# Zoz4/Pooraytracer

Hardware: AMD Instinct MI355X
Metric: Mrays/s (primary+secondary) at fixed spp; s/frame in ms_per_step (higher is better)
Workload: dtype f64; 1 GPU; cornell-box (synthetic stand-in, 20492 tris, 4-wide BVH 6148 nodes) 1024x1024 spp=500 depth=20 rr=0.8 bSampleLights seed=1; parallelism=32x32 tiles dealt diagonally over 1 GPU(s), rays_per_frame=2362685805

## Files before the change

pooraytracer_amd/csrc/prt_device.h:

```cpp
#pragma once
#include <hip/hip_runtime.h>
#include <stdint.h>

#include "prt_types.h"
#include "prt_light_pick.h"

#define PRT_DEV __device__ __forceinline__
typedef prt_real real;
#define PRT_F32 (sizeof(prt_real) == 4)
#define RL(x) ((real)(x))
template <typename R> struct real4_of;
template <> struct real4_of<double> { typedef double4 type; };
template <> struct real4_of<float> { typedef float4 type; };
typedef real4_of<real>::type real4;
#define PRT_NOCUR ((int32_t)0x80000000)
#ifndef PRT_BOX_PK
#define PRT_BOX_PK 1
#endif
#ifndef PRT_LEAF_BATCH
#define PRT_LEAF_BATCH 32
#endif
#ifndef PRT_INNER_MIN
#define PRT_INNER_MIN 12
#endif

struct d3 {
    real x, y, z;
};
struct d2 {
    real x, y;
};
PRT_DEV d3 mk3(real x, real y, real z) { return d3{x, y, z}; }
PRT_DEV d3 ld3(const real* p) { return d3{p[0], p[1], p[2]}; }
PRT_DEV d3 operator+(d3 a, d3 b) { return {a.x + b.x, a.y + b.y, a.z + b.z}; }
PRT_DEV d3 operator-(d3 a, d3 b) { return {a.x - b.x, a.y - b.y, a.z - b.z}; }
PRT_DEV d3 operator-(d3 a) { return {-a.x, -a.y, -a.z}; }
PRT_DEV d3 operator*(d3 a, d3 b) { return {a.x * b.x, a.y * b.y, a.z * b.z}; }
PRT_DEV d3 operator*(d3 a, real s) { return {a.x * s, a.y * s, a.z * s}; }
PRT_DEV d3 operator*(real s, d3 a) { return {s * a.x, s * a.y, s * a.z}; }
PRT_DEV d3 operator/(d3 a, real s);
PRT_DEV real dot(d3 a, d3 b) { return a.x * b.x + a.y * b.y + a.z * b.z; }
PRT_DEV d3 cross(d3 x, d3 y) { return {x.y * y.z - y.y * x.z, x.z * y.x - y.z * x.x, x.x * y.y - y.x * x.y}; }
PRT_DEV double fast_rsqrt(double x) {
    const double y = __builtin_amdgcn_rsq(x);
    const double g = x * y, h = 0.5 * y;
    const double r = fma(-h, g, 0.5);
    const double h1 = fma(h, r, h), g1 = fma(g, r, g);
    const double e = fma(-h1, g1, 0.5);
    return 2.0 * fma(h1, e, h1);
}
PRT_DEV double fast_sqrt(double x) {
    const double y = __builtin_amdgcn_rsq(x);
    const double g = x * y, h = 0.5 * y;
    const double r = fma(-h, g, 0.5);
    const double g1 = fma(g, r, g), h1 = fma(h, r, h);
    const double d = fma(-g1, g1, x);
    const double s = fma(d, h1, g1);
    return x == 0.0 ? 0.0 : s;
}
PRT_DEV double fast_rcp(double b) {
    double r = __builtin_amdgcn_rcp(b);
    r = fma(fma(-b, r, 1.0), r, r);
    r = fma(fma(-b, r, 1.0), r, r);
    return r;
}
PRT_DEV double fast_div(double a, double b) {
    const double r = fast_rcp(b);
    const double q = a * r;
    return fma(fma(-b, q, a), r, q);
}
PRT_DEV float fast_rsqrt(float x) { return __builtin_amdgcn_rsqf(x); }
PRT_DEV float fast_sqrt(float x) { return __builtin_amdgcn_sqrtf(x); }
PRT_DEV float fast_rcp(float b) { return __builtin_amdgcn_rcpf(b); }
PRT_DEV float fast_div(float a, float b) { return a * __builtin_amdgcn_rcpf(b); }
PRT_DEV double ieee_sqrt(double x) { return sqrt(x); }
PRT_DEV float ieee_sqrt(float x) { return __builtin_amdgcn_sqrtf(x); }
PRT_DEV double ieee_div(double a, double b) { return a / b; }
PRT_DEV float ieee_div(float a, float b) { return a * __builtin_amdgcn_rcpf(b); }
PRT_DEV d3 operator/(d3 a, real s) {
    const real r = fast_rcp(s);
    return {a.x * r, a.y * r, a.z * r};
}
PRT_DEV real length(d3 v) { return fast_sqrt(dot(v, v)); }
PRT_DEV d3 normalize(d3 v) { return v * fast_rsqrt(dot(v, v)); }
PRT_DEV d3 normalize_len(d3 v, real& len) {
    const real q = dot(v, v);
    const real inv = fast_rsqrt(q);
    len = q * inv;
    return v * inv;
}

#define PRT_PI RL(3.14159265358979323846)
#define PRT_INV_PI RL(0.31830988618379067154)
#define PRT_INV_2PI RL(0.15915494309189533577)
#define PRT_PI_OVER_2 RL(1.57079632679489661923)
#define PRT_PI_OVER_4 RL(0.78539816339744830961)
#define PRT_INF RL(__builtin_huge_val())

PRT_DEV uint64_t mix64(uint64_t z) {
    z ^= z >> 30;
    z *= 0xBF58476D1CE4E5B9ULL;
    z ^= z >> 27;
    z *= 0x94D049BB133111EBULL;
    z ^= z >> 31;
    return z;
}
PRT_DEV uint64_t seed_key(uint64_t seed) { return mix64(seed + 0x9E3779B97F4A7C15ULL); }
struct Rng {
    uint64_t s;
    PRT_DEV void seed_keyed(uint64_t key, uint64_t pixel, uint64_t sample) {
        s = mix64(((uint64_t)((uint32_t)(key >> 32) ^ (uint32_t)(pixel + 1)) << 32) | ((uint32_t)key ^ (uint32_t)(sample + 1)));
        if (s == 0) s = 0x9E3779B97F4A7C15ULL;
    }
    PRT_DEV void seed(uint64_t seed, uint64_t pixel, uint64_t sample) { seed_keyed(seed_key(seed), pixel, sample); }
    PRT_DEV real next() {
        uint32_t s0 = (uint32_t)s, s1 = (uint32_t)(s >> 32);
        const uint32_t r = s0 * 0x9E3779BBu;
        s1 ^= s0;
        s0 = __builtin_amdgcn_alignbit(s0, s0, 6) ^ s1 ^ (s1 << 9);
        s1 = __builtin_amdgcn_alignbit(s1, s1, 19);
        s = ((uint64_t)s1 << 32) | s0;
        if (PRT_F32) return (real)(r >> 8) * RL(5.9604644775390625e-8);
        return (real)(r >> 1) * (RL(1.0) / RL(2147483648.0));
    }
};

struct HitInfo {
    real t;
    real alpha, beta;
    int32_t tri;
};

struct WorkCount {
    uint32_t nodes, tris;
    uint32_t tris_full;
    uint32_t inner_rounds, leaf_rounds;
};

template <bool PAD>
PRT_DEV const DTri* tri_at(const DScene& S, uint32_t i) {
    return reinterpret_cast<const DTri*>(reinterpret_cast<const char*>(S.tris) + (size_t)i * (PAD ? PRT_TRI_PAD_STRIDE(real) : (uint32_t)sizeof(DTri)));
}

PRT_DEV bool tri_test(const DTri* __restrict__ T, d3 o, d3 d, real tmin, real tmax, real& t_out, real& a_out,
                      real& b_out, const real4* pre = nullptr, uint32_t* n_full = nullptr) {
    const real4* q = reinterpret_cast<const real4*>(T);
    real4 q0 = pre ? *pre : q[0], q1 = q[1];
    d3 n = mk3(q0.x, q0.y, q0.z);
    real denom = dot(n, d);
    if (fabs(denom) < RL(1e-8)) return false;
    real t = ieee_div(q0.w - dot(n, o), denom);
    if (!(tmin <= t && t <= tmax)) return false;
    if (n_full) ++*n_full;
    const real4 q2 = q[2];
    const d3 p = o + d * t;
    const real alpha = (p.x * q1.x + p.y * q1.y + p.z * q1.z) - q1.w;
    const real beta = (p.x * q2.x + p.y * q2.y + p.z * q2.z) - q2.w;
    if (alpha != alpha || beta != beta) return false;
    if ((alpha < 0) || (beta < 0) || (alpha + beta > 1)) return false;
    t_out = t;
    a_out = alpha;
    b_out = beta;
    return true;
}

PRT_DEV float f32_up(real x) {
    const float f = (float)x;
    return f + fabsf(f) * 2.4e-7f;
}
PRT_DEV float f32_down(real x) {
    const float f = (float)x;
    return f - fabsf(f) * 2.4e-7f;
}

struct SlabAxis {
    float idq, c_lo, c_hi;
    uint32_t rot;
};
PRT_DEV SlabAxis slab_axis(real o, real d, float E, float g0, float gs) {
    SlabAxis a;
    const float df = (float)d;
    float id = __builtin_amdgcn_rcpf(df);
    if (!(fabsf(id) <= 1e28f)) id = copysignf(1e28f, df);
    const float r = (float)((real)g0 - o);
    const float c = r * id;
    const float pad = fmaf(E, fabsf(id), fabsf(c)) * 9.5367432e-7f;
    a.idq = gs * id;
    a.c_lo = c - pad;
    a.c_hi = c + pad;
    a.rot = id >= 0.f ? 0u : 16u;
    return a;
}

template <bool PAD, bool PK = false>
struct Trav {
    d3 o, d;
    real tmin;
    HitInfo hit;
    SlabAxis ax, ay, az;
    float tminf, tbestf;
    int32_t cur;
    int32_t sp;
    bool active;

    PRT_DEV void init(const DScene& S, d3 o_, d3 d_, real tmin_, real tmax_) {
        o = o_;
        d = d_;
        start(S, tmin_, tmax_);
    }
    PRT_DEV void start(const DScene& S, real tmin_, real tmax_) {
        tmin = tmin_;
        ax = slab_axis(o.x, d.x, S.slab_scale, S.grid_origin[0], S.grid_step[0]);
        ay = slab_axis(o.y, d.y, S.slab_scale, S.grid_origin[1], S.grid_step[1]);
        az = slab_axis(o.z, d.z, S.slab_scale, S.grid_origin[2], S.grid_step[2]);
        tminf = f32_down(tmin_);
        tbestf = f32_up(tmax_);
        hit.t = tmax_;
        hit.tri = -1;
        sp = 0;
        cur = 0;
        active = S.n_tris != 0;
    }

    PRT_DEV void box4(uint32_t x, uint32_t y, uint32_t z, float& n, float& f) const {
        x = __builtin_amdgcn_alignbit(x, x, ax.rot);
        y = __builtin_amdgcn_alignbit(y, y, ay.rot);
        z = __builtin_amdgcn_alignbit(z, z, az.rot);
        float nx, fx, ny, fy, nz, fz;
        if (PK) {
        typedef float f2_ __attribute__((ext_vector_type(2)));
        const f2_ tx = __builtin_elementwise_fma(f2_{(float)(x & 0xffffu), (float)(x >> 16)}, f2_{ax.idq, ax.idq}, f2_{ax.c_lo, ax.c_hi});
        const f2_ ty = __builtin_elementwise_fma(f2_{(float)(y & 0xffffu), (float)(y >> 16)}, f2_{ay.idq, ay.idq}, f2_{ay.c_lo, ay.c_hi});
        const f2_ tz = __builtin_elementwise_fma(f2_{(float)(z & 0xffffu), (float)(z >> 16)}, f2_{az.idq, az.idq}, f2_{az.c_lo, az.c_hi});
        nx = tx.x, fx = tx.y, ny = ty.x, fy = ty.y, nz = tz.x, fz = tz.y;
        } else {
        nx = fmaf((float)(x & 0xffffu), ax.idq, ax.c_lo), fx = fmaf((float)(x >> 16), ax.idq, ax.c_hi);
        ny = fmaf((float)(y & 0xffffu), ay.idq, ay.c_lo), fy = fmaf((float)(y >> 16), ay.idq, ay.c_hi);
        nz = fmaf((float)(z & 0xffffu), az.idq, az.c_lo), fz = fmaf((float)(z >> 16), az.idq, az.c_hi);
        }
        n = fmaxf(fmaxf(fmaxf(nx, ny), nz), tminf);
        f = fminf(fminf(fminf(fx, fy), fz), tbestf);
    }
    template <bool COUNT>
    PRT_DEV void inner_step(const DScene& S, uint32_t* stk, WorkCount& wc) {
        const uint4* np = reinterpret_cast<const uint4*>(S.nodes + cur);
        const uint4 bx = np[0], by = np[1], bz = np[2], rf = np[3];
        if (COUNT) wc.nodes++;
        float n0, f0, n1, f1, n2, f2, n3, f3;
        box4(bx.x, by.x, bz.x, n0, f0);
        box4(bx.y, by.y, bz.y, n1, f1);
        box4(bx.z, by.z, bz.z, n2, f2);
        box4(bx.w, by.w, bz.w, n3, f3);
        uint32_t k0 = n0 <= f0 ? __float_as_uint(n0) : 0xffffffffu;
        uint32_t k1 = n1 <= f1 ? __float_as_uint(n1) : 0xffffffffu;
        uint32_t k2 = (n2 <= f2 && rf.z != 0x80000000u) ? __float_as_uint(n2) : 0xffffffffu;
        uint32_t k3 = (n3 <= f3 && rf.w != 0x80000000u) ? __float_as_uint(n3) : 0xffffffffu;
        uint32_t r0 = rf.x, r1 = rf.y, r2 = rf.z, r3 = rf.w;
#define PRT_CE(ka, ra, kb, rb)                  \
    {                                           \
        const bool sw_ = kb < ka;               \
        const uint32_t tk_ = sw_ ? kb : ka;     \
        kb = sw_ ? ka : kb;                     \
        ka = tk_;                               \
        const uint32_t tr_ = sw_ ? rb : ra;     \
        rb = sw_ ? ra : rb;                     \
        ra = tr_;                               \
    }
        PRT_CE(k0, r0, k1, r1)
        PRT_CE(k2, r2, k3, r3)
        PRT_CE(k0, r0, k2, r2)
        PRT_CE(k1, r1, k3, r3)
        PRT_CE(k1, r1, k2, r2)
#undef PRT_CE
        if (k3 != 0xffffffffu) {
            stk[sp * 64] = r3;
            sp++;
        }
        if (k2 != 0xffffffffu) {
            stk[sp * 64] = r2;
            sp++;
        }
        if (k1 != 0xffffffffu) {
            stk[sp * 64] = r1;
            sp++;
        }
        if (k0 != 0xffffffffu) {
            cur = (int32_t)r0;
        } else if (sp == 0) {
            cur = PRT_NOCUR;
        } else {
            sp--;
            cur = (int32_t)stk[sp * 64];
        }
        if (cur == PRT_NOCUR) active = false;
    }

    template <bool COUNT>
    PRT_DEV bool test_leaf(const DScene& S, int32_t ref, WorkCount& wc, real tmin_use, bool any_hit) {
        const uint32_t enc = ~(uint32_t)ref;
        const uint32_t first = enc >> 3, cnt = (enc & 7u) + 1u;
        bool stop = false;
        real4 q0n = *reinterpret_cast<const real4*>(tri_at<PAD>(S, first));
        for (uint32_t i = 0; i < cnt; ++i) {
            real t, al, be;
            if (COUNT) wc.tris++;
            const real4 q0c = q0n;
            if (i + 1 < cnt) q0n = *reinterpret_cast<const real4*>(tri_at<PAD>(S, first + i + 1));
            if (tri_test(tri_at<PAD>(S, first + i), o, d, tmin_use, hit.t, t, al, be, &q0c, COUNT ? &wc.tris_full : nullptr)) {
                hit.t = t;
                if (!any_hit) {
                    hit.alpha = al;
                    hit.beta = be;
                }
                hit.tri = (int32_t)(first + i);
                tbestf = f32_up(t);
                if (any_hit) stop = true;
            }
        }
        return stop;
    }

    template <bool COUNT>
    PRT_DEV void leaf_step(const DScene& S, uint32_t* stk, WorkCount& wc, real tmin_use, bool any_hit) {
        bool stop = false;
        if (cur < 0 && cur != PRT_NOCUR) {
            stop = test_leaf<COUNT>(S, cur, wc, tmin_use, any_hit);
            cur = PRT_NOCUR;
        }
        if (stop) {
            active = false;
        } else if (cur == PRT_NOCUR) {
            if (sp == 0) active = false;
            else {
                sp--;
                cur = (int32_t)stk[sp * 64];
            }
        }
    }

    template <bool COUNT>
    PRT_DEV void round(const DScene& S, uint32_t* stk, WorkCount& wc, int leaf_batch, int inner_min, real tmin_use,
                       bool any_hit) {
        if (COUNT && __ballot(active && cur >= 0) != 0ULL) wc.inner_rounds++;
        if (active && cur >= 0) inner_step<COUNT>(S, stk, wc);
        const bool parked = active && cur < 0;
        const bool has_leaf = active && cur < 0 && cur != PRT_NOCUR;
        const int n_parked = __popcll(__ballot(parked));
        const int n_inner = __popcll(__ballot(active && cur >= 0));
        if (n_parked >= leaf_batch || n_inner <= inner_min) {
            if (COUNT && __ballot(has_leaf) != 0ULL) wc.leaf_rounds++;
            if (has_leaf) leaf_step<COUNT>(S, stk, wc, tmin_use, any_hit);
        }
    }
};

PRT_DEV int wave_count(bool p) { return __popcll(__ballot(p)); }

#define PRT_TEX_QUAD_REALS 16
template <bool EXTRA, bool NARROW = false>
PRT_DEV d3 tex_value(const DScene& S, int ti, real u, real v) {
    const DTexture tx = S.textures[ti];
    if (!tx.has_data) return mk3(RL(0.), RL(1.), RL(1.));
    u = fmin(fmax(u, RL(0.0)), RL(1.0));
    v = fmin(fmax(v, RL(0.0)), RL(1.0));
    real x = u * (tx.width - RL(1.));
    real y = (RL(1.) - v) * (tx.height - RL(1.));
    int x0 = (int)x, y0 = (int)y;
    real fx = x - x0, fy = y - y0;
    d3 c00, c10, c01, c11;
    if (!EXTRA || !S.tex_compact) {
        const real4* q = reinterpret_cast<const real4*>(S.texels_lin + tx.offset + (size_t)(y0 * tx.width + x0) * PRT_TEX_QUAD_REALS);
        if (NARROW) {
            const real4 r0 = q[0], r1 = q[1];
            const d3 top = mk3(r0.x, r0.y, r0.z) * (1 - fx) + mk3(r0.w, r1.x, r1.y) * fx;
            __builtin_amdgcn_sched_barrier(0);
            const real4 r2 = q[2];
            const d3 bot = mk3(r1.z, r1.w, r2.x) * (1 - fx) + mk3(r2.y, r2.z, r2.w) * fx;
            return top * (1 - fy) + bot * fy;
        }
        const real4 q0 = q[0], q1 = q[1], q2 = q[2];
        c00 = mk3(q0.x, q0.y, q0.z), c10 = mk3(q0.w, q1.x, q1.y);
        c01 = mk3(q1.z, q1.w, q2.x), c11 = mk3(q2.y, q2.z, q2.w);
    } else {
        const int x1 = min(x0 + 1, tx.width - 1), y1 = min(y0 + 1, tx.height - 1);
        const real* base = S.texels_lin + tx.offset;
        if (NARROW) {
            const d3 top = ld3(base + ((size_t)y0 * tx.width + x0) * 3) * (1 - fx) + ld3(base + ((size_t)y0 * tx.width + x1) * 3) * fx;
            __builtin_amdgcn_sched_barrier(0);
            const d3 bot = ld3(base + ((size_t)y1 * tx.width + x0) * 3) * (1 - fx) + ld3(base + ((size_t)y1 * tx.width + x1) * 3) * fx;
            return top * (1 - fy) + bot * fy;
        }
        c00 = ld3(base + ((size_t)y0 * tx.width + x0) * 3), c10 = ld3(base + ((size_t)y0 * tx.width + x1) * 3);
        c01 = ld3(base + ((size_t)y1 * tx.width + x0) * 3), c11 = ld3(base + ((size_t)y1 * tx.width + x1) * 3);
    }
    d3 c0 = c00 * (1 - fx) + c10 * fx;
    d3 c1 = c01 * (1 - fx) + c11 * fx;
    return c0 * (1 - fy) + c1 * fy;
}

PRT_DEV double fma_ks(double a, double b, double k) {
#if defined(__HIP_DEVICE_COMPILE__)
    double r;
    asm("v_fma_f64 %0, %1, %2, %3" : "=v"(r) : "v"(a), "v"(b), "s"(k));
    return r;
#else
    return __builtin_fma(a, b, k);
#endif
}
PRT_DEV float fma_ks(float a, float b, float k) { return __builtin_fmaf(a, b, k); }
PRT_DEV double fma_sk(double a, double k, double c) {
#if defined(__HIP_DEVICE_COMPILE__)
    double r;
    asm("v_fma_f64 %0, %1, %2, %3" : "=v"(r) : "v"(a), "s"(k), "v"(c));
    return r;
#else
    return __builtin_fma(a, k, c);
#endif
}
PRT_DEV double mul_ks(double a, double k) {
#if defined(__HIP_DEVICE_COMPILE__)
    double r;
    asm("v_mul_f64 %0, %1, %2" : "=v"(r) : "v"(a), "s"(k));
    return r;
#else
    return a * k;
#endif
}

PRT_DEV void sincos_quarter(real x, real& sn, real& cs) {
    const real z = x * x;
    if (PRT_F32) {
        sn = x + (x * z) * (RL(-1.6666667e-01) + z * (RL(8.3333333e-03) + z * (RL(-1.9841270e-04) + z * RL(2.7557319e-06))));
        cs = RL(1.0) + z * (RL(-0.5) + z * (RL(4.1666667e-02) + z * (RL(-1.3888889e-03) + z * RL(2.4801587e-05))));
        return;
    }
    real ps = fma_ks(z, RL(1.58969099521155010221e-10), -RL(2.50507602534068634195e-08));
    ps = fma_ks(z, ps, RL(2.75573137070700676789e-06));
    ps = fma_ks(z, ps, -RL(1.98412698298579493134e-04));
    ps = fma_ks(z, ps, RL(8.33333333332248946124e-03));
    sn = x + (x * z) * fma_ks(z, ps, -RL(1.66666666666666324348e-01));
    real pc = fma_ks(z, -RL(1.13596475577881948265e-11), RL(2.08757232129817482790e-09));
    pc = fma_ks(z, pc, -RL(2.75573143513906633035e-07));
    pc = fma_ks(z, pc, RL(2.48015872894767294178e-05));
    pc = fma_ks(z, pc, -RL(1.38888888888741095749e-03));
    pc = z * fma_ks(z, pc, RL(4.16666666666666019037e-02));
    cs = RL(1.0) - (RL(0.5) * z - z * pc);
}
PRT_DEV void sincos_turns(real u, real& sn, real& cs) {
    const real k = floor(RL(4.0) * u + RL(0.5));
    const real r = u - RL(0.25) * k;
    real s, c;
    sincos_quarter(RL(2.0) * PRT_PI * r, s, c);
    const int q = (int)k & 3;
    sn = (q == 0) ? s : (q == 1) ? c : (q == 2) ? -s : -c;
    cs = (q == 0) ? c : (q == 1) ? -s : (q == 2) ? -c : s;
}
PRT_DEV void sincos_any(double theta, double, double& sn, double& cs) { sincos(theta, &sn, &cs); }
PRT_DEV void sincos_any(float, float u, float& sn, float& cs) {
    sn = __builtin_amdgcn_sinf(u);
    cs = __builtin_amdgcn_cosf(u);
}
PRT_DEV d2 disk_concentric(d2 u) {
    d2 off = {RL(2.) * u.x - RL(1.), RL(2.) * u.y - RL(1.)};
    if (off.x == RL(0.) && off.y == RL(0.)) return {RL(0.), RL(0.)};
    real sn, cs;
    if (fabs(off.x) > fabs(off.y)) {
        sincos_quarter(PRT_PI_OVER_4 * fast_div(off.y, off.x), sn, cs);
        return {off.x * cs, off.x * sn};
    }
    sincos_quarter(PRT_PI_OVER_4 * fast_div(off.x, off.y), cs, sn);
    return {off.y * cs, off.y * sn};
}
PRT_DEV d3 cosine_hemisphere(Rng& rng) {
    real first = rng.next();
    real second = rng.next();
    d2 dd = disk_concentric(d2{second, first});
    real z = fast_sqrt(fmax(RL(0.0), RL(1.) - dd.x * dd.x - dd.y * dd.y));
    return mk3(dd.x, dd.y, z);
}
// ... 333 lines not shown
```

pooraytracer_amd/csrc/prt_kernels.hip:

```cpp
#include <hip/hip_runtime.h>

#include <type_traits>

#include "../../include/prt.h"
#include "prt_device.h"
#include "prt_launch.h"

#ifndef PRT_F32_TU
#define PRT_F32_TU 0
#endif
#if PRT_F32_TU
#define PRT_NS prt32
#else
#define PRT_NS prt
#endif
#define PRT_DYN_STACK PRT_F32_TU

#ifndef PRT_RENDER_WAVES
#define PRT_RENDER_WAVES 2
#endif
#ifndef PRT_RENDER_WAVES_LEAN
#define PRT_RENDER_WAVES_LEAN 3
#endif
#ifndef PRT_RENDER_WAVES_TEX
// ... 292 lines not shown
    unsigned long long c = wave_sum((unsigned long long)wc.tris);
    unsigned long long f = wave_sum((unsigned long long)wc.tris_full);
    if (lane == 0) {
        atomicAdd(&ctr->rays_closest, a);
        if (COUNT) {
            atomicAdd(&ctr->node_fetches, b);
            atomicAdd(&ctr->tri_tests, c);
            atomicAdd(&ctr->tri_full, f);
        }
    }
}

template <int PARK_STRIDE>
PRT_DEV void park_real(uint32_t* base, int word, real v) {
    if (PRT_F32) {
        base[word * PARK_STRIDE] = __float_as_uint((float)v);
    } else {
        const unsigned long long b = (unsigned long long)__double_as_longlong((double)v);
        base[word * PARK_STRIDE] = (uint32_t)b;
        base[(word + 1) * PARK_STRIDE] = (uint32_t)(b >> 32);
    }
}
template <int PARK_STRIDE>
PRT_DEV real unpark_real(const uint32_t* base, int word) {
    if (PRT_F32) return (real)__uint_as_float(base[word * PARK_STRIDE]);
    return (real)__longlong_as_double((long long)(((unsigned long long)base[(word + 1) * PARK_STRIDE] << 32) | base[word * PARK_STRIDE]));
}
#define PRT_RW ((int)(sizeof(real) / 4))
#define PARK_T 0
#define PARK_TRI PRT_RW
#define PARK_DIR (PRT_RW + 1)
#define PARK_DIR_GLOBAL(feat) (((feat) & PRT_FEAT_TEX) != 0)
#define PARK_AB_AT(feat) (PARK_DIR_GLOBAL(feat) ? PRT_RW + 1 : 4 * PRT_RW + 1)
#define PARK_WORDS(feat) (((feat) & PRT_FEAT_TEX) ? 3 * PRT_RW + 1 : 4 * PRT_RW + 1)

PRT_DEV void load_ray(const void* ray_list, uint32_t i, d3& o, d3& d) {
    const PrtRay* r = static_cast<const PrtRay*>(ray_list) + i;
    o = mk3((real)r->o[0], (real)r->o[1], (real)r->o[2]);
    d = mk3((real)r->d[0], (real)r->d[1], (real)r->d[2]);
}

template <typename R>
struct RenderArgsT {
    DSceneT<R> S;
    DCameraT<R> C;
    DRenderParamsT<R> P;
    double* partial;
    DCounters* ctr;
};
typedef RenderArgsT<real> RenderArgs;
typedef const RenderArgs __attribute__((address_space(4)))* ColdRenderArgs;
PRT_DEV ColdRenderArgs cold_args() {
    ColdRenderArgs q = (ColdRenderArgs)__builtin_amdgcn_kernarg_segment_ptr();
    asm volatile("" : "+s"(q));
    return q;
}

template <bool COUNT, int FEAT, bool LLDS, bool PAD>
__global__ __launch_bounds__(PRT_BLOCK, render_waves(FEAT)) void k_render(RenderArgs A) {
    const DScene& S = A.S;
    const DRenderParams& P = A.P;
    DCounters* const ctr = A.ctr;
    constexpr bool RAYS = (FEAT & PRT_FEAT_RAYS) != 0;
    __shared__ uint32_t s_qoff[PRT_BLOCK / 64];
    __shared__ unsigned long long s_rays[PRT_BLOCK / 64];
    __shared__ real s_center[4];
    constexpr int NPARK = PRT_BLOCK;
    __shared__ uint32_t s_park[PARK_WORDS(FEAT)][NPARK];
#define park (&s_park[0][threadIdx.x])
    const int lane = threadIdx.x & 63, wave = threadIdx.x >> 6;
    extern __shared__ __align__(16) unsigned char s_dyn_all[];
#if PRT_DYN_STACK
    uint32_t* stk = reinterpret_cast<uint32_t*>(s_dyn_all) + (size_t)(wave * P.stack_depth) * 64 + lane;
    unsigned char* s_dyn = s_dyn_all + (size_t)(PRT_BLOCK / 64) * P.stack_depth * 64 * sizeof(uint32_t);
#else
    __shared__ uint32_t s_stack[PRT_BLOCK / 64][PRT_STACK_DEPTH][64];
    uint32_t* stk = &s_stack[wave][0][lane];
    unsigned char* s_dyn = s_dyn_all;
#endif
    if (lane == 0) {
        s_qoff[wave] = 0;
        s_rays[wave] = 0ULL;
    }
    if (threadIdx.x < 3) s_center[threadIdx.x] = A.C.center[threadIdx.x];
    if (!LLDS) __syncthreads();
    const DLightNode* lds_lights = reinterpret_cast<const DLightNode*>(s_dyn);
    const DMaterial* lds_mats = reinterpret_cast<const DMaterial*>(s_dyn + (size_t)P.light_lds * sizeof(DLightNode));
    const DLightTri* lds_ltris = reinterpret_cast<const DLightTri*>(s_dyn + (size_t)P.light_lds * sizeof(DLightNode) + (size_t)P.mat_lds * sizeof(DMaterial));
    if (LLDS) {
        uint4* dst = reinterpret_cast<uint4*>(s_dyn);
        const uint4* src = reinterpret_cast<const uint4*>(S.light_nodes);
        for (int i = threadIdx.x; i < P.light_lds; i += PRT_BLOCK) dst[i] = src[i];
        dst += P.light_lds;
        src = reinterpret_cast<const uint4*>(S.materials);
        const int nm = P.mat_lds * (int)(sizeof(DMaterial) / 16);
        for (int i = threadIdx.x; i < nm; i += PRT_BLOCK) dst[i] = src[i];
        dst += nm;
        src = reinterpret_cast<const uint4*>(S.light_tris);
        const int nl = P.ltri_lds * (int)(sizeof(DLightTri) / 16);
        for (int i = threadIdx.x; i < nl; i += PRT_BLOCK) dst[i] = src[i];
        __syncthreads();
    }
#define MATERIAL(i) (LLDS ? lds_mats[(i)] : S.materials[(i)])
    d3 pst_[2];
#define PST_LD(k) (pst_[(k) / 3])
#define PST_ST(k, v) (pst_[(k) / 3] = (v))
#define S_ACC 0
#define S_BETA 3
#define ADD_RADIANCE(x) PST_ST(S_ACC, PST_LD(S_ACC) + (PST_LD(S_BETA) * (x)) * inv_spp)
#define TRACING (COUNT && P.scramble == PRT_ITEMS_FROM_LIST && ctr->trace != nullptr)
#define TRACE_VERTEX(prim_)                                                     \
    do {                                                                        \
        if (TRACING) {                                                          \
            const int v_ = P.max_depth - depth;                                 \
            if (v_ < PRT_TRACE_VERTS) {                                         \
                int32_t* tw_ = ctr->trace + (size_t)item * PRT_TRACE_WORDS;     \
                tw_[0] = v_ + 1;                                                \
                tw_[1 + 2 * v_] = (prim_);                                      \
                tw_[2 + 2 * v_] = 0;                                            \
            }                                                                   \
        }                                                                       \
    } while (0)
#define TRACE_FLAG_AT(v_, bit_)                                                 \
    do {                                                                        \
        if (TRACING) {                                                          \
            if ((v_) < PRT_TRACE_VERTS) ctr->trace[(size_t)item * PRT_TRACE_WORDS + 2 + 2 * (v_)] |= (bit_); \
        }                                                                       \
    } while (0)
#define TRACE_FLAG(bit_)                                                        \
    do {                                                                        \
        if (TRACING) {                                                          \
            const int v_ = P.max_depth - depth;                                 \
            if (v_ < PRT_TRACE_VERTS) ctr->trace[(size_t)item * PRT_TRACE_WORDS + 2 + 2 * v_] |= (bit_); \
        }                                                                       \
    } while (0)

    WorkCount wc{0, 0, 0, 0, 0};
    uint32_t n_refills = 0;

    int state = ST_FETCH;
    uint32_t item = 0;
    int px = 0, py = 0, s = 0, s_end = 0, depth = 0;
    uint32_t pixel = 0;
    bool first = true, prev_skip = false;
    PST_ST(S_ACC, mk3(0, 0, 0));
    PST_ST(S_BETA, mk3(1, 1, 1));
    d3 rd = mk3(0, 0, 1);
    int32_t sh_tri = -1;
    real ldist = 0;
    int32_t ltri = 0;
    constexpr bool ONE_PASS = PRT_ONE_PASS_VERTEX && !(FEAT & (PRT_FEAT_PHONG | PRT_FEAT_TEX));
    constexpr bool EVAL_FLAT = ONE_PASS && !(FEAT & PRT_FEAT_CT);
    constexpr bool TURN = ONE_PASS && PRT_SAMPLE_TURNOVER && !(PRT_F32 && !(FEAT & PRT_FEAT_CT));
    d3 pending = mk3(0, 0, 0);
    d3 next_d = mk3(0, 0, 1);
    bool cont = false;
    int nee_v = 0;
    Rng rng;
    rng.s = 0;
    const real inv_spp = RL(1.0) / (real)P.spp;
    Trav<PAD, PRT_BOX_PK != 0> tr;
    tr.init(S, mk3(0, 0, 0), rd, RL(0.0), RL(0.0));
    tr.hit.alpha = tr.hit.beta = RL(0.0);
    tr.active = false;

#if PRT_K3_PROFILE
    unsigned long long prof_[6] = {0, 0, 0, 0, 0, 0}, prof_t_ = __builtin_readcyclecounter();
#endif
#define END_OF_SAMPLE(next) do {                                                                                                                                          \
        const d3 acc = PST_LD(S_ACC);                                                                                                                                     \
        s++;                                                                                                                                                              \
        if (s < s_end) state = (next);                                                                                                                                     \
        else {                                                                                                                                                            \
            double* o = cold_args()->partial + (size_t)item * 3;                                                                                                          \
            o[0] = (double)acc.x;                                                                    \
            o[1] = (double)acc.y;                                                                                                                                         \
            o[2] = (double)acc.z;                                                                                                                                         \
            state = ST_FETCH;                                                                                                                                             \
        }                                                                                                                                                                 \
    } while (0)
#define NEW_SAMPLE(parked) do {                                                                                                                                           \
                                                                                                                            \
        rng.seed_keyed(P.seed_key, (uint64_t)pixel, (uint64_t)s);                                                                                                         \
        if (!RAYS && P.jitter) {                                                                                                                                          \
                                                           \
                                                                                                                      \
            const ColdRenderArgs q = cold_args();                                                                                                                         \
            const int W = q->C.width;                                                                                                                                     \
            const int jy = (int)(pixel / (uint32_t)W), jx = (int)(pixel - (uint32_t)jy * (uint32_t)W);                                                                    \
            const real fy = (real)jy + (rng.next() - RL(0.5));                                                                                                            \
            const real fx = (real)jx + (rng.next() - RL(0.5));                                                                                                            \
            const d3 ps = mk3(q->C.pixel00[0], q->C.pixel00[1], q->C.pixel00[2]) + fx * mk3(q->C.du[0], q->C.du[1], q->C.du[2]) +                                         \
                          fy * mk3(q->C.dv[0], q->C.dv[1], q->C.dv[2]);                                                                                                   \
            tr.o = mk3(q->C.center[0], q->C.center[1], q->C.center[2]);                                                                                                   \
            tr.d = ps - tr.o;                                                                                                                                             \
            state = ST_CLOSEST;                                                                                                                                           \
        } else {                                                                                                                                                          \
                                                        \
                                                 \
                                                        \
            if (RAYS) {                                                                          \
                load_ray(ctr->ray_list, (uint32_t)px, tr.o, tr.d);                                                                                                        \
            } else if (PARK_DIR_GLOBAL(FEAT)) {                                               \
                tr.o = mk3(s_center[0], s_center[1], s_center[2]);                                                                                                        \
                const ColdRenderArgs q = cold_args();                                                                                                                     \
                const d3 ps = mk3(q->C.pixel00[0], q->C.pixel00[1], q->C.pixel00[2]) + (real)px * mk3(q->C.du[0], q->C.du[1], q->C.du[2]) +                               \
                              (real)py * mk3(q->C.dv[0], q->C.dv[1], q->C.dv[2]);                                                                                         \
                tr.d = ps - tr.o;                                                                                                                                         \
            } else {                                                                                                                                                      \
                tr.o = mk3(s_center[0], s_center[1], s_center[2]);                                                                                                        \
                tr.d = mk3(unpark_real<NPARK>(park, PARK_DIR), unpark_real<NPARK>(park, PARK_DIR + PRT_RW), unpark_real<NPARK>(park, PARK_DIR + 2 * PRT_RW));             \
            }                                                                                                                                                             \
            tr.hit.t = unpark_real<NPARK>(park, PARK_T);                                                                                                                  \
            tr.hit.tri = (int32_t)park[PARK_TRI * NPARK];                                                                                                                 \
            if (FEAT & PRT_FEAT_TEX) {                                                                                                                                    \
                tr.hit.alpha = unpark_real<NPARK>(park, PARK_AB_AT(FEAT));                                                                                                \
                tr.hit.beta = unpark_real<NPARK>(park, PARK_AB_AT(FEAT) + PRT_RW);                                                                                        \
            }                                                                                                                                                             \
            state = (parked);                                                                                                                                             \
        }                                                                                                                                                                 \
        PST_ST(S_BETA, mk3(1, 1, 1));                                                                                                                                     \
        depth = P.max_depth;                                                                                                                                              \
        first = true;                                                                                                                                                     \
        prev_skip = false;                                                                                                                                                \
    } while (0)
    for (;;) {
        if (COUNT) n_refills++;
        PROF_MARK(0);
        int started = 0;
        if (!tr.active) {
            bool end_sample = false, do_scatter = false;
            bool nee = false;
            bool have_fr = false;
            d3 fr_seen = mk3(0, 0, 0);
            if (state == ST_PRIMARY) {
                bool flat = false;
                d3 x = mk3(0, 0, 0);
                if ((FEAT & (PRT_FEAT_PHONG | PRT_FEAT_CT)) && P.scramble != PRT_ITEMS_FROM_LIST) {
                    if (tr.hit.tri < 0) {
                        const ColdRenderArgs q = cold_args();
                        x = mk3(q->P.background[0], q->P.background[1], q->P.background[2]);
                        flat = true;
                    } else {
                        const DMaterial& m = MATERIAL(S.shade[tr.hit.tri].material);
                        if (m.has_emission) {
                            x = ld3(m.emission);
                            flat = true;
                        }
                    }
                }
                if (flat) {
                    const d3 term = (mk3(1, 1, 1) * x) * inv_spp;
                    d3 acc = PST_LD(S_ACC);
                    for (; s < s_end; ++s) acc = acc + term;
                    double* o = cold_args()->partial + (size_t)item * 3;
                    o[0] = (double)acc.x;
                    o[1] = (double)acc.y;
                    o[2] = (double)acc.z;
                    state = ST_FETCH;
                }
            }
            if (state == ST_PRIMARY) {
                park_real<NPARK>(park, PARK_T, tr.hit.t);
                park[PARK_TRI * NPARK] = (uint32_t)tr.hit.tri;
                if (FEAT & PRT_FEAT_TEX) {
                    park_real<NPARK>(park, PARK_AB_AT(FEAT), tr.hit.alpha);
                    park_real<NPARK>(park, PARK_AB_AT(FEAT) + PRT_RW, tr.hit.beta);
                }
                state = ST_NEW_SAMPLE;
            }
            bool hit_ready = false;
            if (TURN) {
                bool ended = false;
                if (state == ST_CACHED) state = ST_NEW_SAMPLE;
                else if (state == ST_SHADOW) {
                    if (tr.hit.tri < 0) {
                        PST_ST(S_ACC, PST_LD(S_ACC) + pending);
                        TRACE_FLAG_AT(nee_v, PRT_TRACE_VISIBLE);
                    }
                    if (cont) {
                        tr.d = next_d;
                        state = ST_CLOSEST;
                    } else {
                        ended = true;
                    }
                } else if (state == ST_CLOSEST) {
                    if (tr.hit.tri < 0) {
                        if (first || !P.sample_lights) {
                            const ColdRenderArgs q = cold_args();
                            ADD_RADIANCE(mk3(q->P.background[0], q->P.background[1], q->P.background[2]));
                        }
                        TRACE_VERTEX(-1);
                        ended = true;
                    } else {
                        hit_ready = true;
                    }
                }
                if (ended) END_OF_SAMPLE(ST_NEW_SAMPLE);
                if (state == ST_NEW_SAMPLE) {
                    NEW_SAMPLE(ST_CLOSEST);
                    hit_ready = RAYS || !P.jitter;
                }
                PROF_MARK(3);
            } else {
                if (state == ST_CACHED) state = ST_CLOSEST;
            }
// ... 132 lines not shown
                        const real cosTB = -dot(ln, tr.d);
                        const d3 direct = (emission * fr) * fast_div(cosT * cosTB, (ldist * ldist) * pdf);
                        pending = (PST_LD(S_BETA) * direct) * inv_spp;
                    }
                    if (rr_ok) {
                        d3 att;
                        TRACE_FLAG(PRT_TRACE_ROULETTE);
                        if (mat_scatter<FEAT>(S, m, rd, c.f, c.uv, rng, att, next_d)) {
                            TRACE_FLAG(PRT_TRACE_SCATTER);
                            depth--;
                            if (depth >= 0) {
                                const d3 beta = (PST_LD(S_BETA) * att) * P.inv_rr;
                                PST_ST(S_BETA, beta);
                                if (!(beta.x == RL(0.) && beta.y == RL(0.) && beta.z == RL(0.))) {
                                    prev_skip = m.skip_light_sampling != 0;
                                    first = false;
                                    end_sample = false;
                                }
                            }
                        }
                    }
                }
                if (nee) {
                    cont = !end_sample;
                    end_sample = false;
                    state = ST_SHADOW;
                } else if (!end_sample) {
                    tr.d = next_d;
                }
            } else if (do_scatter) {
                end_sample = true;
                if (rng.next() < P.rr) {
                    const ShadeCtx c = make_ctx<FEAT, PAD>(S, rd, tr.hit.alpha, tr.hit.beta, sh_tri);
                    const DMaterial& m = MATERIAL(c.material);
                    d3 att, wi;
                    TRACE_FLAG(PRT_TRACE_ROULETTE);
                    if (mat_scatter<FEAT>(S, m, rd, c.f, c.uv, rng, att, wi, have_fr, fr_seen)) {
                        TRACE_FLAG(PRT_TRACE_SCATTER);
                        depth--;
                        if (depth >= 0) {
                            const d3 beta = (PST_LD(S_BETA) * att) * P.inv_rr;
                            PST_ST(S_BETA, beta);
                            if (!(beta.x == RL(0.) && beta.y == RL(0.) && beta.z == RL(0.))) {
                                tr.d = wi;
                                prev_skip = m.skip_light_sampling != 0;
                                first = false;
                                end_sample = false;
                            }
                        }
                    }
                }
            }
            PROF_MARK(2);
            if (end_sample) END_OF_SAMPLE(TURN ? ST_CACHED : ST_NEW_SAMPLE);

            if (state == ST_FETCH) {
                const ColdRenderArgs q = cold_args();
                const uint32_t n_items = (uint32_t)q->P.n_items;
                {
                    uint32_t off = __builtin_amdgcn_readfirstlane(s_qoff[wave]);
                    item = n_items;
                    while (off < (uint32_t)PRT_ITEM_QUEUES) {
                        const uint32_t qi = (blockIdx.x + off) % (uint32_t)PRT_ITEM_QUEUES;
                        const unsigned long long idx = atomicAdd(&ctr->queue[qi * PRT_QUEUE_STRIDE], 1ULL);
                        const unsigned long long it = ((idx >> 6) * PRT_ITEM_QUEUES + qi) * 64ULL + (idx & 63ULL);
                        if (it < n_items) {
                            item = (uint32_t)it;
                            break;
                        }
                        ++off;
                    }
                    atomicMax(&s_qoff[wave], off);
                }
                if (item >= n_items) {
                    state = ST_DONE;
                } else {
                    const uint32_t ipc = (uint32_t)q->P.items_per_chunk;
                    const uint32_t chunk = item / ipc;
                    const uint32_t oi = item - chunk * ipc;
                    const int W = q->C.width;
                    bool valid;
                    if (RAYS) {
                        px = (int)oi;
                        valid = true;
                    } else if (P.scramble == PRT_ITEMS_FROM_LIST) {
                        const int32_t pix = ctr->pixel_list[oi];
                        py = pix / W;
                        px = pix - py * W;
                        valid = true;
                        if (COUNT && ctr->trace != nullptr) ctr->trace[(size_t)item * PRT_TRACE_WORDS] = 0;
                    } else {
                        valid = tile_pixel(P.scramble, ipc, q->P.tile, q->P.tiles_x, q->P.n_tiles, q->P.rank, q->P.nranks, W, q->C.height, oi, px, py);
                    }
                    if (valid) {
                        s = q->P.chunk_begin[chunk];
                        s_end = q->P.chunk_begin[chunk + 1];
                        if (RAYS) {
                            const uint32_t* keys = ctr->key_list;
                            pixel = keys ? keys[oi] : oi;
                        } else {
                            pixel = (uint32_t)(py * W + px);
                        }
                        PST_ST(S_ACC, mk3(0, 0, 0));
                        if (s >= s_end) {
                            double* o = q->partial + (size_t)item * 3;
                            o[0] = o[1] = o[2] = 0.0;
                        } else if (RAYS) {
                            load_ray(ctr->ray_list, oi, tr.o, tr.d);
                            state = ST_PRIMARY;
                        } else if (P.jitter) {
                            state = TURN ? ST_CACHED : ST_NEW_SAMPLE;
                        } else {
                            const d3 ps = mk3(q->C.pixel00[0], q->C.pixel00[1], q->C.pixel00[2]) + (real)px * mk3(q->C.du[0], q->C.du[1], q->C.du[2]) +
                                          (real)py * mk3(q->C.dv[0], q->C.dv[1], q->C.dv[2]);
                            tr.o = mk3(q->C.center[0], q->C.center[1], q->C.center[2]);
                            tr.d = ps - tr.o;
                            if (!PARK_DIR_GLOBAL(FEAT)) {
                                park_real<NPARK>(park, PARK_DIR, tr.d.x);
                                park_real<NPARK>(park, PARK_DIR + PRT_RW, tr.d.y);
                                park_real<NPARK>(park, PARK_DIR + 2 * PRT_RW, tr.d.z);
                            }
                            state = ST_PRIMARY;
                        }
                    }
                }
            }
            if (!TURN && state == ST_NEW_SAMPLE) NEW_SAMPLE(ST_CACHED);
            PROF_MARK(3);
            if (state == ST_CLOSEST || state == ST_SHADOW || state == ST_PRIMARY) {
                const bool sh_ray = state == ST_SHADOW;
                started = sh_ray ? 2 : 1;
                if (COUNT && ctr->ray_dump != nullptr) {
                    const unsigned long long k = atomicAdd(&ctr->ray_dump_n, 1ULL);
                    if (k < ctr->ray_dump_cap) {
                        PrtRay r;
                        r.o[0] = (double)tr.o.x; r.o[1] = (double)tr.o.y; r.o[2] = (double)tr.o.z;
                        r.d[0] = (double)tr.d.x; r.d[1] = (double)tr.d.y; r.d[2] = (double)tr.d.z;
                        r.tmin = sh_ray ? 0.001 : 0.0001;
                        r.tmax = sh_ray ? (double)(ldist - RL(0.001)) : __builtin_huge_val();
                        static_cast<PrtRay*>(ctr->ray_dump)[k] = r;
                    }
                }
                tr.start(S, sh_ray ? RL(0.001) : RL(0.0001), sh_ray ? ldist - RL(0.001) : PRT_INF);
            }
        }
        PROF_MARK(4);
        {
            const unsigned long long nc = (unsigned long long)__popcll(__ballot(started == 1)), ns = (unsigned long long)__popcll(__ballot(started == 2));
            if (lane == 0) atomicAdd(&s_rays[wave], nc | (ns << 32));
        }
        if (__ballot(state != ST_DONE) == 0ULL) break;
        if (wave_count(state == ST_CACHED) >= P.cached_min) continue;

        do {
            tr.template round<COUNT>(S, stk, wc, P.leaf_batch, P.inner_min, state == ST_SHADOW ? RL(0.001) : RL(0.0001), state == ST_SHADOW);
            if (ONE_PASS) {
                const bool fin = !tr.active && state == ST_SHADOW && cont;
                const int n_fin = wave_count(fin);
                if (n_fin >= P.chain_min) {
                    PROF_MARK(0);
                    if (fin) {
                        if (tr.hit.tri < 0) {
                            PST_ST(S_ACC, PST_LD(S_ACC) + pending);
                            TRACE_FLAG_AT(nee_v, PRT_TRACE_VISIBLE);
                        }
                        tr.d = next_d;
                        state = ST_CLOSEST;
                        if (COUNT && ctr->ray_dump != nullptr) {
                            const unsigned long long k = atomicAdd(&ctr->ray_dump_n, 1ULL);
                            if (k < ctr->ray_dump_cap) {
                                PrtRay r;
                                r.o[0] = (double)tr.o.x; r.o[1] = (double)tr.o.y; r.o[2] = (double)tr.o.z;
                                r.d[0] = (double)tr.d.x; r.d[1] = (double)tr.d.y; r.d[2] = (double)tr.d.z;
                                r.tmin = 0.0001;
                                r.tmax = __builtin_huge_val();
                                static_cast<PrtRay*>(ctr->ray_dump)[k] = r;
                            }
                        }
                        tr.start(S, RL(0.0001), PRT_INF);
                    }
                    if (lane == 0) atomicAdd(&s_rays[wave], (unsigned long long)n_fin);
                    PROF_MARK(5);
                }
            }
        } while (wave_count(tr.active) > P.keep);
    }

    unsigned long long d = wave_sum((unsigned long long)wc.nodes);
    unsigned long long e = wave_sum((unsigned long long)wc.tris);
    unsigned long long f = wave_sum((unsigned long long)wc.tris_full);
    if (lane == 0) {
        const unsigned long long rays = s_rays[wave];
        atomicAdd(&ctr->rays_closest, rays & 0xffffffffULL);
        atomicAdd(&ctr->rays_shadow, rays >> 32);
        if (COUNT) {
            atomicAdd(&ctr->tri_full, f);
#if PRT_K3_PROFILE
            atomicAdd(&ctr->node_fetches, prof_[5]);
            atomicAdd(&ctr->tri_tests, prof_[0]);
            atomicAdd(&ctr->inner_rounds, prof_[1]);
            atomicAdd(&ctr->leaf_rounds, prof_[2]);
            atomicAdd(&ctr->refills, prof_[3]);
            atomicAdd(&ctr->tri_full, prof_[4]);
#else
            atomicAdd(&ctr->node_fetches, d);
            atomicAdd(&ctr->tri_tests, e);
            atomicAdd(&ctr->inner_rounds, (unsigned long long)wc.inner_rounds);
            atomicAdd(&ctr->leaf_rounds, (unsigned long long)wc.leaf_rounds);
            atomicAdd(&ctr->refills, (unsigned long long)n_refills);
#endif
        }
    }
}

#if !PRT_F32_TU
PRT_DEV void chunk_sum(const DRenderParams& P, const double* __restrict__ partial, uint64_t oi, double& r, double& g, double& b) {
    r = 0, g = 0, b = 0;
    for (int c = 0; c < P.chunks; ++c) {
        const double* p = partial + ((uint64_t)c * P.items_per_chunk + oi) * 3;
        r += p[0];
        g += p[1];
        b += p[2];
    }
}

__global__ void k_finalize(DCamera C, DRenderParams P, const double* __restrict__ partial, double* __restrict__ out64,
                           float* __restrict__ out32) {
    const uint64_t oi = (uint64_t)blockIdx.x * blockDim.x + threadIdx.x;
    if (oi >= P.items_per_chunk) return;
    int px, py;
    if (!owned_to_pixel(P, C, oi, px, py)) return;
    double r, g, b;
    chunk_sum(P, partial, oi, r, g, b);
    const size_t m = ((size_t)py * C.width + px) * 3;
    if (out64) {
        out64[m] = r;
        out64[m + 1] = g;
        out64[m + 2] = b;
    }
    if (out32) {
        out32[m] = (float)r;
        out32[m + 1] = (float)g;
        out32[m + 2] = (float)b;
    }
}

__global__ void k_finalize_rays(DRenderParams P, const double* __restrict__ partial, double* __restrict__ out64, float* __restrict__ out32) {
    const uint64_t i = (uint64_t)blockIdx.x * blockDim.x + threadIdx.x;
    if (i >= P.items_per_chunk) return;
    double r, g, b;
    chunk_sum(P, partial, i, r, g, b);
    if (out64) {
        out64[i * 3] = r;
        out64[i * 3 + 1] = g;
        out64[i * 3 + 2] = b;
    }
    if (out32) {
        out32[i * 3] = (float)r;
        out32[i * 3 + 1] = (float)g;
        out32[i * 3 + 2] = (float)b;
    }
}

__global__ void k_accumulate(DCamera C, DRenderParams P, const double* __restrict__ partial, double* __restrict__ sum) {
    const uint64_t oi = (uint64_t)blockIdx.x * blockDim.x + threadIdx.x;
    if (oi >= P.items_per_chunk) return;
    int px, py;
    if (!owned_to_pixel(P, C, oi, px, py)) return;
    double r, g, b;
    chunk_sum(P, partial, oi, r, g, b);
    const size_t m = ((size_t)py * C.width + px) * 3;
    sum[m] += r;
    sum[m + 1] += g;
    sum[m + 2] += b;
}

__global__ void k_sample_lights(DScene S, const double* __restrict__ origins, size_t n, uint64_t seed,
                                PrtLightSample* __restrict__ out) {
    const size_t i = (size_t)blockIdx.x * blockDim.x + threadIdx.x;
    if (i >= n) return;
    Rng rng;
    rng.seed(seed, i, 0);
    const LightPick lp = sample_lights<false, true>(S, mk3(origins[i * 3], origins[i * 3 + 1], origins[i * 3 + 2]), rng);
    PrtLightSample o;
    o.position[0] = lp.pos.x; o.position[1] = lp.pos.y; o.position[2] = lp.pos.z;
    o.normal[0] = lp.n.x; o.normal[1] = lp.n.y; o.normal[2] = lp.n.z;
    o.pdf = lp.pdf;
    o.prim = S.light_tris[lp.tri].prim;
    o.front = lp.front ? 1 : 0;
    out[i] = o;
}

__global__ void k_material_eval(DScene S, int material, const double* __restrict__ wi, const double* __restrict__ wo,
                                const double* __restrict__ uv, size_t n, uint64_t seed, double* __restrict__ out) {
    const size_t i = (size_t)blockIdx.x * blockDim.x + threadIdx.x;
    if (i >= n) return;
    Rng rng;
    rng.seed(seed, i, 0);
    const d2 t = uv ? d2{uv[i * 2], uv[i * 2 + 1]} : d2{0., 0.};
    const d3 f = mat_eval<PRT_FEAT_ALL | PRT_FEAT_EXTRA>(S, S.materials[material], ld3(wi + i * 3), ld3(wo + i * 3), t, rng);
    out[i * 3] = f.x; out[i * 3 + 1] = f.y; out[i * 3 + 2] = f.z;
}
__global__ void k_material_scatter(DScene S, int material, const double* __restrict__ rd, d3 normal, d3 tangent,
                                   const double* __restrict__ uv, size_t n, uint64_t seed, double* __restrict__ wi_out,
                                   double* __restrict__ att_out, int32_t* __restrict__ ok_out) {
    const size_t i = (size_t)blockIdx.x * blockDim.x + threadIdx.x;
// ... 482 lines not shown
```

Before: 12840 Mrays/s.

## Restructure f64 traversal loop with ballot masks and software-pipelined leaf tests

For the f64 one-pass path, replaces the generic round/ballot traversal loop with a version that computes lane masks once per iteration and derives activity from the current node instead of a separate active flag. It cuts redundant ballots and branch work in the inner loop. It also adds a leaf tester that double-buffers triangle record loads and uses FMA-based dot products with a fused barycentric reject test. FMA ordering can change rounding of hit results, and the restructured control flow could diverge subtly from the original loop semantics.

```diff
diff --git a/pooraytracer_amd/csrc/prt_device.h b/pooraytracer_amd/csrc/prt_device.h
--- a/pooraytracer_amd/csrc/prt_device.h
+++ b/pooraytracer_amd/csrc/prt_device.h
@@ -163,6 +163,29 @@
     b_out = beta;
     return true;
 }
+
+PRT_DEV real dot_yxz(real ax, real ay, real az, real bx, real by, real bz) { return fma(az, bz, fma(ax, bx, ay * by)); }
+PRT_DEV bool tri_test_ord(const DTri* __restrict__ T, d3 o, d3 d, real tmin, real tmax, real& t_out, real& a_out,
+                          real& b_out, const real4& q0, uint32_t* n_full) {
+    const real4* q = reinterpret_cast<const real4*>(T);
+    real4 q1 = q[1];
+    real denom = dot_yxz(q0.x, q0.y, q0.z, d.x, d.y, d.z);
+    if (fabs(denom) < RL(1e-8)) return false;
+    real t = ieee_div(q0.w - dot_yxz(q0.x, q0.y, q0.z, o.x, o.y, o.z), denom);
+    if (!(tmin <= t && t <= tmax)) return false;
+    if (n_full) ++*n_full;
+    const real4 q2 = q[2];
+    const d3 p = mk3(fma(d.x, t, o.x), fma(d.y, t, o.y), fma(d.z, t, o.z));
+    const real alpha = dot_yxz(p.x, p.y, p.z, q1.x, q1.y, q1.z) - q1.w;
+    const real beta = dot_yxz(p.x, p.y, p.z, q2.x, q2.y, q2.z) - q2.w;
+    if (!(alpha >= 0 && beta >= 0 && alpha + beta <= 1)) return false;
+    t_out = t;
+    a_out = alpha;
+    b_out = beta;
+    return true;
+}
+
+PRT_DEV unsigned long long lane_mask(bool p) { return __builtin_amdgcn_ballot_w64(p); }
 
 PRT_DEV float f32_up(real x) {
     const float f = (float)x;
@@ -321,10 +344,47 @@
     }
 
     template <bool COUNT>
+    PRT_DEV bool test_leaf_pp(const DScene& S, int32_t ref, WorkCount& wc, real tmin_use, bool any_hit) {
+        const uint32_t enc = ~(uint32_t)ref;
+        const uint32_t first = enc >> 3, cnt = (enc & 7u) + 1u;
+        constexpr uint32_t STRIDE = PAD ? PRT_TRI_PAD_STRIDE(real) : (uint32_t)sizeof(DTri);
+        const char* rec = reinterpret_cast<const char*>(tri_at<PAD>(S, first));
+        bool stop = false;
+        uint32_t i = 0;
+        auto test = [&](const real4& q0) {
+            real t, al, be;
+            if (COUNT) wc.tris++;
+            if (tri_test_ord(reinterpret_cast<const DTri*>(rec), o, d, tmin_use, hit.t, t, al, be, q0, COUNT ? &wc.tris_full : nullptr)) {
+                hit.t = t;
+                if (!any_hit) {
+                    hit.alpha = al;
+                    hit.beta = be;
+                }
+                hit.tri = (int32_t)(first + i);
+                tbestf = f32_up(t);
+                if (any_hit) stop = true;
+            }
+        };
+        real4 qa = *reinterpret_cast<const real4*>(rec), qb;
+        for (;;) {
+            if (i + 1 < cnt) qb = *reinterpret_cast<const real4*>(rec + STRIDE);
+            test(qa);
+            if (++i == cnt) break;
+            rec += STRIDE;
+            if (i + 1 < cnt) qa = *reinterpret_cast<const real4*>(rec + STRIDE);
+            test(qb);
+            if (++i == cnt) break;
+            rec += STRIDE;
+        }
+        return stop;
+    }
+
+    template <bool COUNT, bool PP = false>
     PRT_DEV void leaf_step(const DScene& S, uint32_t* stk, WorkCount& wc, real tmin_use, bool any_hit) {
         bool stop = false;
         if (cur < 0 && cur != PRT_NOCUR) {
-            stop = test_leaf<COUNT>(S, cur, wc, tmin_use, any_hit);
+            if constexpr (PP) stop = test_leaf_pp<COUNT>(S, cur, wc, tmin_use, any_hit);
+            else stop = test_leaf<COUNT>(S, cur, wc, tmin_use, any_hit);
             cur = PRT_NOCUR;
         }
         if (stop) {
diff --git a/pooraytracer_amd/csrc/prt_kernels.hip b/pooraytracer_amd/csrc/prt_kernels.hip
--- a/pooraytracer_amd/csrc/prt_kernels.hip
+++ b/pooraytracer_amd/csrc/prt_kernels.hip
@@ -468,6 +468,7 @@
     constexpr bool ONE_PASS = PRT_ONE_PASS_VERTEX && !(FEAT & (PRT_FEAT_PHONG | PRT_FEAT_TEX));
     constexpr bool EVAL_FLAT = ONE_PASS && !(FEAT & PRT_FEAT_CT);
     constexpr bool TURN = ONE_PASS && PRT_SAMPLE_TURNOVER && !(PRT_F32 && !(FEAT & PRT_FEAT_CT));
+    constexpr bool WAVE_DIET = ONE_PASS && !PRT_F32;
     d3 pending = mk3(0, 0, 0);
     d3 next_d = mk3(0, 0, 1);
     bool cont = false;
@@ -906,6 +907,55 @@
         if (__ballot(state != ST_DONE) == 0ULL) break;
         if (wave_count(state == ST_CACHED) >= P.cached_min) continue;
 
+        if constexpr (WAVE_DIET) {
+            bool sh = state == ST_SHADOW;
+            unsigned long long m_chain = lane_mask(sh && cont);
+            unsigned long long m_act;
+            if (!tr.active) tr.cur = PRT_NOCUR;
+            do {
+                if (COUNT && lane_mask(tr.cur >= 0) != 0ULL) wc.inner_rounds++;
+                if (tr.cur >= 0) tr.template inner_step<COUNT>(S, stk, wc);
+                const unsigned long long m_inner = lane_mask(tr.cur >= 0);
+                const unsigned long long m_parked = lane_mask((uint32_t)tr.cur > (uint32_t)PRT_NOCUR);
+                m_act = m_inner | m_parked;
+                if (__popcll(m_parked) >= P.leaf_batch || __popcll(m_inner) <= P.inner_min) {
+                    if (COUNT && m_parked != 0ULL) wc.leaf_rounds++;
+                    if ((uint32_t)tr.cur > (uint32_t)PRT_NOCUR) tr.template leaf_step<COUNT, !COUNT>(S, stk, wc, sh ? RL(0.001) : RL(0.0001), sh);
+                    m_act = lane_mask(tr.cur != PRT_NOCUR);
+                }
+                const unsigned long long m_fin = m_chain & ~m_act;
+                if (__popcll(m_fin) >= P.chain_min) {
+                    PROF_MARK(0);
+                    if (tr.cur == PRT_NOCUR && sh && cont) {
+                        if (tr.hit.tri < 0) {
+                            PST_ST(S_ACC, PST_LD(S_ACC) + pending);
+                            TRACE_FLAG_AT(nee_v, PRT_TRACE_VISIBLE);
+                        }
+                        tr.d = next_d;
+                        state = ST_CLOSEST;
+                        sh = false;
+                        if (COUNT && ctr->ray_dump != nullptr) {
+                            const unsigned long long k = atomicAdd(&ctr->ray_dump_n, 1ULL);
+                            if (k < ctr->ray_dump_cap) {
+                                PrtRay r;
+                                r.o[0] = (double)tr.o.x; r.o[1] = (double)tr.o.y; r.o[2] = (double)tr.o.z;
+                                r.d[0] = (double)tr.d.x; r.d[1] = (double)tr.d.y; r.d[2] = (double)tr.d.z;
+                                r.tmin = 0.0001;
+                                r.tmax = __builtin_huge_val();
+                                static_cast<PrtRay*>(ctr->ray_dump)[k] = r;
+                            }
+                        }
+                        tr.start(S, RL(0.0001), PRT_INF);
+                        if (!tr.active) tr.cur = PRT_NOCUR;
+                    }
+                    if (lane == 0) atomicAdd(&s_rays[wave], (unsigned long long)__popcll(m_fin));
+                    m_chain &= m_act;
+                    m_act = lane_mask(tr.cur != PRT_NOCUR);
+                    PROF_MARK(5);
+                }
+            } while (__popcll(m_act) > P.keep);
+            tr.active = tr.cur != PRT_NOCUR;
+        } else
         do {
             tr.template round<COUNT>(S, stk, wc, P.leaf_batch, P.inner_min, state == ST_SHADOW ? RL(0.001) : RL(0.0001), state == ST_SHADOW);
             if (ONE_PASS) {
```

Measured after the change: 13800 Mrays/s, median of 6. 1.08x the previous value.
